# cvg/glue-factory

Hardware: AMD Instinct MI355X
Metric: image-pairs/sec (train step) SP+LightGlue N=2048 d=256 L=9 (higher is better)
Workload: dtype bf16; 1 GPU; configs[1]: SuperPoint + LightGlue train step -- frozen SuperPoint-open forward on 2x32 synthetic 1024x1024 images resident in HBM (view1 = view0 warped by a sampled homography, SURVEY 8(d)(P); first block and the 64-channel 3x3 blocks as fused HIP kernels, library convolutions + fused HIP tails for the 128/256-channel blocks), homography ground truth (gf_gt_nn), LightGlue fwd + loss + bwd + fused; pairs_per_gpu=32, global_batch=32, keypoints=2048, descriptor_dim=256, layers=9, parallelism=dp1

## Files before the change

glue-factory_amd/csrc/conv3x3.hip:

```cpp
#include "gf_common.h"
#include "gf_amd.h"

#ifndef C3_ABL
#define C3_ABL 0
#endif

namespace {

typedef unsigned int u32x4 __attribute__((ext_vector_type(4)));
typedef unsigned int u32x2 __attribute__((ext_vector_type(2)));
typedef __attribute__((address_space(3))) void c3_lds_void;
typedef const __attribute__((address_space(1))) void c3_glb_void;

constexpr int C3_TH = 8, C3_TW = 32;
constexpr int C3_IW = C3_TW + 2, C3_IH = C3_TH + 2;
constexpr int C3_NPIX = C3_IW * C3_IH;
constexpr int C3_PIECES = 44;
constexpr int C3_INBUF = C3_PIECES * 1024;
constexpr int C3_OUT = C3_TH * C3_TW * 128;
constexpr int C3_STAGE = 2 * C3_INBUF;
constexpr int C3_CST = C3_STAGE + 2 * C3_OUT;
constexpr int C3_LDS = C3_CST + 3 * 64 * 4;
#ifndef C3_AGPR_FRAGS_V
#define C3_AGPR_FRAGS_V 48
#endif
constexpr int C3_AGPR_FRAGS = C3_AGPR_FRAGS_V;

template <int OFF> __device__ __forceinline__ u32x4 c3_rd128(unsigned a) {
    u32x4 v;
    asm volatile("ds_read_b128 %0, %1 offset:%2" : "=v"(v) : "v"(a), "n"(OFF) : "memory");
    return v;
}
template <int N> __device__ __forceinline__ void c3_wait_lgkm() { asm volatile("s_waitcnt lgkmcnt(%0)" ::"n"(N) : "memory"); }
template <int N> __device__ __forceinline__ void c3_wait_vm() { asm volatile("s_waitcnt vmcnt(%0)" ::"n"(N) : "memory"); }
template <typename V> __device__ __forceinline__ void c3_tie(V& v) { asm volatile("" : "+v"(v)); }

struct C3Params {
    const bf16_t* x; const bf16_t* w;
    const float* bias; const float* scale; const float* shift;
    bf16_t* y;
    int ldy;
    int B, H, W, relu;
};

template <bool POOL, bool RELU>
__global__ __launch_bounds__(256, 1) void conv3x3_c64_kernel(C3Params p) {
    extern __shared__ __attribute__((aligned(1024))) char smem[];
    const unsigned lds0 = (unsigned)(size_t)smem;
    const int lane = threadIdx.x & 63, wave = __builtin_amdgcn_readfirstlane(threadIdx.x >> 6);
    const int l31 = lane & 31, hi = lane >> 5;
    const int tx_n = p.W / C3_TW, ty_n = p.H / C3_TH;
    const int tiles = tx_n * ty_n * p.B;
#ifndef C3_SKEW32
#define C3_SKEW32 5
#endif
    const int skew = tx_n % 32 == 0 ? C3_SKEW32 : 0;

    bf16x8 wf[2][9][4];
#pragma unroll
    for (int nt = 0; nt < 2; ++nt)
#pragma unroll
        for (int t = 0; t < 9; ++t)
#pragma unroll
            for (int ks = 0; ks < 4; ++ks) {
                const bf16x8 v = *reinterpret_cast<const bf16x8*>(p.w + ((t * 64 + 32 * nt + l31) * 64 + 16 * ks + 8 * hi));
                {
                    wf[nt][t][ks] = v;
                    if ((nt * 9 + t) * 4 + ks < C3_AGPR_FRAGS) asm volatile("" : "+a"(wf[nt][t][ks]));
                    else asm volatile("" : "+v"(wf[nt][t][ks]));
                }
            }
    float* cst = reinterpret_cast<float*>(smem + C3_CST);
    if (threadIdx.x < 64) {
        cst[threadIdx.x] = p.bias[threadIdx.x];
        cst[64 + threadIdx.x] = p.scale[threadIdx.x];
        cst[128 + threadIdx.x] = p.shift[threadIdx.x];
    }

    struct Tile { int b, y0, x0; };
    auto coords = [&](int tile) {
        Tile t;
        t.b = tile / (tx_n * ty_n);
        const int r = tile - t.b * (tx_n * ty_n);
        const int ty = r / tx_n;
        const int tx = (r - ty * tx_n + skew * ty) % tx_n;
        t.y0 = ty * C3_TH; t.x0 = tx * C3_TW;
        return t;
    };
    const int pc_pp0 = wave * 8 + (lane >> 3);
    const int pc_lane0 = pc_pp0 * 128 + ((lane & 7) ^ ((pc_pp0 >> 1) & 7)) * 16;
    const int pc_wrap = (p.W - C3_IW) * 128;
    int pc_off = 0, pc_ix = 0;
    auto image_rsrc = [&](const Tile& t) {
        return __builtin_amdgcn_make_buffer_rsrc((void*)(p.x + (int64_t)t.b * p.H * p.W * 64), 0, p.H * p.W * 128, 0x00020000);
    };
    auto issue_piece = [&](__amdgpu_buffer_rsrc_t rs, const Tile& t, int buf, int i) {
        if (i == 0) { pc_ix = pc_pp0; pc_off = ((t.y0 - 1) * p.W + t.x0 - 1) * 128 + pc_lane0; }
        __builtin_amdgcn_raw_ptr_buffer_load_lds(rs, (c3_lds_void*)(smem + buf * C3_INBUF + (wave + 4 * i) * 1024), 16, pc_off, 0, 0, 0);
        const bool wrap = pc_ix >= C3_IW - 32;
        pc_off += 32 * 128 + (wrap ? pc_wrap : 0);
        pc_ix += wrap ? 32 - C3_IW : 32;
    };
    auto zero_halo = [&](const Tile& t, int buf) {
        for (int pp = threadIdx.x; pp < C3_NPIX; pp += 256) {
            const int iy = pp / C3_IW, ix = pp - iy * C3_IW;
            const int gy = t.y0 - 1 + iy, gx = t.x0 - 1 + ix;
            if (gy < 0 || gy >= p.H || gx < 0 || gx >= p.W) {
                u32x4 z = {0u, 0u, 0u, 0u};
#pragma unroll
                for (int c = 0; c < 8; ++c) *reinterpret_cast<u32x4*>(smem + buf * C3_INBUF + pp * 128 + c * 16) = z;
            }
        }
    };
    auto is_border = [&](const Tile& t) {
        return t.y0 == 0 || t.x0 == 0 || t.y0 == p.H - C3_TH || t.x0 == p.W - C3_TW;
    };

    constexpr int NSTORE = POOL ? 4 : 8;
    const int st_off0 = POOL ? ((int)(threadIdx.x >> 7) * (p.W / 2) + ((int)(threadIdx.x >> 3) & 15)) * p.ldy + ((int)threadIdx.x & 7) * 8
                             : ((int)(threadIdx.x >> 3)) * p.ldy + ((int)threadIdx.x & 7) * 8;
    auto store_addr = [&](const Tile& t, int k) -> bf16_t* {
        if (!POOL) {
            bf16_t* base = p.y + (((int64_t)t.b * p.H + t.y0 + k) * p.W + t.x0) * p.ldy;
            return base + st_off0;
        }
        bf16_t* base = p.y + (((int64_t)t.b * (p.H / 2) + t.y0 / 2 + 2 * k) * (p.W / 2) + t.x0 / 2) * p.ldy;
        return base + st_off0;
    };
    auto stage_at = [&](int sb, int opx, int c) { return C3_STAGE + sb * C3_OUT + opx * 128 + ((c ^ ((opx >> 1) & 7)) << 4); };
    u32x4 sv[POOL ? 2 : 1];
    float pm[POOL ? 8 : 1];
    auto store_read = [&](int sb, int k) {
        if (!POOL) {
            const int u = threadIdx.x + 256 * k;
            sv[0] = c3_rd128<0>(lds0 + stage_at(sb, u >> 3, u & 7));
        } else {
            const int u = threadIdx.x + 256 * (k >> 1);
            const int py = u >> 7, px = (u >> 3) & 15, c = u & 7;
#pragma unroll
            for (int d = 0; d < 2; ++d) sv[d] = c3_rd128<0>(lds0 + stage_at(sb, (2 * py + (k & 1)) * C3_TW + 2 * px + d, c));
        }
    };
    auto store_write = [&](const Tile& t, int k) {
        if (!POOL) {
            c3_tie(sv[0]);
            if (!(C3_ABL & 8)) *reinterpret_cast<u32x4*>(store_addr(t, k)) = sv[0];
        } else {
#pragma unroll
            for (int d = 0; d < 2; ++d) {
                c3_tie(sv[d]);
                const bf16x8 vv = __builtin_bit_cast(bf16x8, sv[d]);
#pragma unroll
                for (int e = 0; e < 8; ++e) pm[e] = (d || (k & 1)) ? fmaxf(pm[e], (float)vv[e]) : (float)vv[e];
            }
            if (k & 1) {
                const bf16x8 o = {(bf16_t)pm[0], (bf16_t)pm[1], (bf16_t)pm[2], (bf16_t)pm[3],
                                  (bf16_t)pm[4], (bf16_t)pm[5], (bf16_t)pm[6], (bf16_t)pm[7]};
                if (!(C3_ABL & 8)) *reinterpret_cast<bf16x8*>(store_addr(t, k >> 1)) = o;
            }
        }
    };

    unsigned ab[4][3];
#pragma unroll
    for (int ro = 0; ro < 4; ++ro)
#pragma unroll
        for (int dx = 0; dx < 3; ++dx) {
            const int pp = (2 * wave + ro) * C3_IW + l31 + dx;
            ab[ro][dx] = lds0 + (unsigned)(pp * 128 + ((hi ^ ((pp >> 1) & 7)) << 4));
        }
    const int T = (tiles - (int)blockIdx.x + (int)gridDim.x - 1) / (int)gridDim.x;
    if (T <= 0) return;
    Tile cur = coords(blockIdx.x), prev = cur;
    {
        const __amdgpu_buffer_rsrc_t rs0 = image_rsrc(cur);
#pragma unroll
        for (int i = 0; i < C3_PIECES / 4; ++i) issue_piece(rs0, cur, 0, i);
    }
    c3_wait_vm<0>();
    asm volatile("s_waitcnt lgkmcnt(0)\n\ts_barrier" ::: "memory");
    if (is_border(cur)) {
        zero_halo(cur, 0);
        asm volatile("s_waitcnt lgkmcnt(0)\n\ts_barrier" ::: "memory");
    }

    for (int i = 0; i < T; ++i) {
        const int buf = i & 1;
        const bool has_next = i + 1 < T;
        const Tile nxt = coords(blockIdx.x + (has_next ? i + 1 : i) * gridDim.x);
        const __amdgpu_buffer_rsrc_t nxt_rs = image_rsrc(nxt);

        f32x16 acc[2][2];
#pragma unroll
        for (int nt = 0; nt < 2; ++nt)
#pragma unroll
            for (int r = 0; r < 2; ++r)
#pragma unroll
                for (int k = 0; k < 16; ++k) acc[nt][r][k] = 0.f;
        auto base = [&](int t, int r) { return ab[r + t / 3][t % 3] + (unsigned)(buf * C3_INBUF); };
        u32x4 ra[4], rb[4];
        if (!(C3_ABL & 4)) {
            const unsigned a = base(0, 0);
#pragma unroll
            for (int ks = 0; ks < 4; ++ks) ra[ks] = c3_rd128<0>(a ^ (32u * ks));
        }
#pragma unroll
        for (int g = 0; g < ((C3_ABL & 4) ? 0 : 18); ++g) {
            const int t = g >> 1, r = g & 1;
            u32x4 (&cur_)[4] = (g & 1) ? rb : ra;
            u32x4 (&nxt_)[4] = (g & 1) ? ra : rb;
            const int k = POOL ? ((g & 3) == 1 && g < 16 ? g >> 2 : -1) : (g >= 1 && g <= 8 ? g - 1 : -1);
            if (k >= 0) store_read(buf ^ 1, k);
            if (g + 1 < 18) {
                const unsigned a = base((g + 1) >> 1, (g + 1) & 1);
#pragma unroll
                for (int ks = 0; ks < 4; ++ks) nxt_[ks] = c3_rd128<0>(a ^ (32u * ks));
                c3_wait_lgkm<4>();
            } else {
                c3_wait_lgkm<0>();
            }
            if (g < C3_PIECES / 4 && !(C3_ABL & 2)) issue_piece(nxt_rs, nxt, buf ^ 1, g);
#pragma unroll
            for (int ks = 0; ks < 4; ++ks) c3_tie(cur_[ks]);
#pragma unroll
            for (int nt = 0; nt < 2; ++nt)
#pragma unroll
                for (int ks = 0; ks < 4; ++ks) {
                    acc[nt][r] = __builtin_amdgcn_mfma_f32_32x32x16_bf16(wf[nt][t][ks], __builtin_bit_cast(bf16x8, cur_[ks]), acc[nt][r], 0, 0, 0);
                }
            if (k >= 0) store_write(prev, k);
        }

        if (C3_ABL & 1) {
#pragma unroll
            for (int r = 0; r < 2; ++r) { asm volatile("" ::"v"(acc[0][r]), "v"(acc[1][r])); }
        } else {
#pragma unroll
            for (int nt = 0; nt < 2; ++nt)
#pragma unroll
                for (int g = 0; g < 4; ++g) {
                    const int c0 = 32 * nt + 8 * g + 4 * hi;
                    const f32x4 cb = *reinterpret_cast<const f32x4*>(cst + c0);
                    const f32x4 cs = *reinterpret_cast<const f32x4*>(cst + 64 + c0);
                    const f32x4 ch = *reinterpret_cast<const f32x4*>(cst + 128 + c0);
#pragma unroll
                    for (int r = 0; r < 2; ++r) {
                        const int opx = (2 * wave + r) * C3_TW + l31;
                        float o[4];
#pragma unroll
                        for (int e = 0; e < 4; ++e) {
                            float a = acc[nt][r][4 * g + e] + cb[e];
                            if (RELU) a = fmaxf(a, 0.f);
                            o[e] = fmaf(a, cs[e], ch[e]);
                        }
                        st4(reinterpret_cast<bf16_t*>(smem + stage_at(buf, opx, 4 * nt + g) + 8 * hi), o[0], o[1], o[2], o[3]);
                    }
                }
        }
        c3_wait_vm<0>();
        asm volatile("s_waitcnt lgkmcnt(0)\n\ts_barrier" ::: "memory");
        if (has_next && is_border(nxt)) {
            zero_halo(nxt, buf ^ 1);
            asm volatile("s_waitcnt lgkmcnt(0)\n\ts_barrier" ::: "memory");
        }
        prev = cur; cur = nxt;
    }
    {
        const int sb = (T - 1) & 1;
#pragma unroll
        for (int k = 0; k < NSTORE; ++k) {
            store_read(sb, k);
            c3_wait_lgkm<0>();
            store_write(prev, k);
        }
    }
}

}

extern "C" int gf_conv3x3_c64_ld(const void* x, const void* w, const float* bias, const float* scale, const float* shift,
                                 void* y, int64_t ldy, int B, int H, int W, int relu, int pool, int dtype, void* stream);
extern "C" int gf_conv3x3_c64(const void* x, const void* w, const float* bias, const float* scale, const float* shift,
                              void* y, int B, int H, int W, int relu, int pool, int dtype, void* stream) {
    return gf_conv3x3_c64_ld(x, w, bias, scale, shift, y, 64, B, H, W, relu, pool, dtype, stream);
}
extern "C" int gf_conv3x3_c64_ld(const void* x, const void* w, const float* bias, const float* scale, const float* shift,
                                 void* y, int64_t ldy, int B, int H, int W, int relu, int pool, int dtype, void* stream) {
    if (B <= 0 || H <= 0 || W <= 0) return GF_ERR_SHAPE;
    if (dtype != GF_BF16) return GF_ERR_DTYPE;
    if (H % C3_TH || W % C3_TW) return GF_ERR_UNSUPPORTED;
    if ((int64_t)H * W * 128 >= (1ll << 31)) return GF_ERR_UNSUPPORTED;
    if (ldy < 64 || ldy % 8) return GF_ERR_ALIGN;
    if ((reinterpret_cast<size_t>(x) | reinterpret_cast<size_t>(w) | reinterpret_cast<size_t>(y)) & 15) return GF_ERR_ALIGN;
    if ((int64_t)H * W * ldy >= (1ll << 31)) return GF_ERR_UNSUPPORTED;
    C3Params p;
    p.x = static_cast<const bf16_t*>(x); p.w = static_cast<const bf16_t*>(w); p.bias = bias; p.scale = scale; p.shift = shift;
    p.y = static_cast<bf16_t*>(y); p.ldy = (int)ldy; p.B = B; p.H = H; p.W = W; p.relu = relu;
    const size_t lds = C3_LDS;
    const int tiles = (W / C3_TW) * (H / C3_TH) * B;
    const int grid = tiles < 256 ? tiles : 256;
    hipStream_t st = reinterpret_cast<hipStream_t>(stream);
    void (*k)(C3Params) = pool ? (relu ? conv3x3_c64_kernel<true, true> : conv3x3_c64_kernel<true, false>)
                               : (relu ? conv3x3_c64_kernel<false, true> : conv3x3_c64_kernel<false, false>);
    hipError_t e = hipFuncSetAttribute(reinterpret_cast<const void*>(k), hipFuncAttributeMaxDynamicSharedMemorySize, (int)lds);
    if (e != hipSuccess) return (int)e;
    k<<<dim3(grid), 256, lds, st>>>(p);
    return (int)hipGetLastError();
}
```

Before: 534.4 image-pairs/s.

## Fuse 2x2 max-pool into conv3x3 epilogue using DPP lane max

For the pooled variant, the 2x2 max-pool now runs in registers inside the epilogue. Vertical max is taken across the two accumulator rows and horizontal max across adjacent lanes via DPP v_max_f32_dpp, and only the pooled result is written to the LDS stage buffer. This quarters stage LDS writes and halves the store loop. The bias/ReLU/scale epilogue math also uses packed f32x2 FMA. It adds inline-asm DPP hazards (s_nop) and changes when pooled stores are issued within the MFMA loop (C3_PG).

Result: no change. 538.7 image-pairs/s, median of 6 (+0.8%).

```diff
diff --git a/glue-factory_amd/csrc/conv3x3.hip b/glue-factory_amd/csrc/conv3x3.hip
--- a/glue-factory_amd/csrc/conv3x3.hip
+++ b/glue-factory_amd/csrc/conv3x3.hip
@@ -21,6 +21,12 @@
 constexpr int C3_STAGE = 2 * C3_INBUF;
 constexpr int C3_CST = C3_STAGE + 2 * C3_OUT;
 constexpr int C3_LDS = C3_CST + 3 * 64 * 4;
+#ifndef C3_PK
+#define C3_PK 1
+#endif
+#ifndef C3_PG
+#define C3_PG 12
+#endif
 #ifndef C3_AGPR_FRAGS_V
 #define C3_AGPR_FRAGS_V 48
 #endif
@@ -34,6 +40,16 @@
 template <int N> __device__ __forceinline__ void c3_wait_lgkm() { asm volatile("s_waitcnt lgkmcnt(%0)" ::"n"(N) : "memory"); }
 template <int N> __device__ __forceinline__ void c3_wait_vm() { asm volatile("s_waitcnt vmcnt(%0)" ::"n"(N) : "memory"); }
 template <typename V> __device__ __forceinline__ void c3_tie(V& v) { asm volatile("" : "+v"(v)); }
+__device__ __forceinline__ void c3_max_lane_xor1(float (&m)[4]) {
+    float r0, r1, r2, r3;
+    asm volatile("s_nop 1\n\t"
+                 "v_max_f32_dpp %0, %4, %4 quad_perm:[1,0,3,2] row_mask:0xf bank_mask:0xf\n\t"
+                 "v_max_f32_dpp %1, %5, %5 quad_perm:[1,0,3,2] row_mask:0xf bank_mask:0xf\n\t"
+                 "v_max_f32_dpp %2, %6, %6 quad_perm:[1,0,3,2] row_mask:0xf bank_mask:0xf\n\t"
+                 "v_max_f32_dpp %3, %7, %7 quad_perm:[1,0,3,2] row_mask:0xf bank_mask:0xf"
+                 : "=&v"(r0), "=&v"(r1), "=&v"(r2), "=&v"(r3) : "v"(m[0]), "v"(m[1]), "v"(m[2]), "v"(m[3]));
+    m[0] = r0; m[1] = r1; m[2] = r2; m[3] = r3;
+}
 
 struct C3Params {
     const bf16_t* x; const bf16_t* w;
@@ -116,7 +132,8 @@
         return t.y0 == 0 || t.x0 == 0 || t.y0 == p.H - C3_TH || t.x0 == p.W - C3_TW;
     };
 
-    constexpr int NSTORE = POOL ? 4 : 8;
+    constexpr int NSTORE = POOL ? 2 : 8;
+    constexpr int OUTB = POOL ? C3_OUT / 4 : C3_OUT;
     const int st_off0 = POOL ? ((int)(threadIdx.x >> 7) * (p.W / 2) + ((int)(threadIdx.x >> 3) & 15)) * p.ldy + ((int)threadIdx.x & 7) * 8
                              : ((int)(threadIdx.x >> 3)) * p.ldy + ((int)threadIdx.x & 7) * 8;
     auto store_addr = [&](const Tile& t, int k) -> bf16_t* {
@@ -127,38 +144,15 @@
         bf16_t* base = p.y + (((int64_t)t.b * (p.H / 2) + t.y0 / 2 + 2 * k) * (p.W / 2) + t.x0 / 2) * p.ldy;
         return base + st_off0;
     };
-    auto stage_at = [&](int sb, int opx, int c) { return C3_STAGE + sb * C3_OUT + opx * 128 + ((c ^ ((opx >> 1) & 7)) << 4); };
-    u32x4 sv[POOL ? 2 : 1];
-    float pm[POOL ? 8 : 1];
+    auto stage_at = [&](int sb, int opx, int c) { return C3_STAGE + sb * OUTB + opx * 128 + ((c ^ ((opx >> 1) & 7)) << 4); };
+    u32x4 sv;
     auto store_read = [&](int sb, int k) {
-        if (!POOL) {
-            const int u = threadIdx.x + 256 * k;
-            sv[0] = c3_rd128<0>(lds0 + stage_at(sb, u >> 3, u & 7));
-        } else {
-            const int u = threadIdx.x + 256 * (k >> 1);
-            const int py = u >> 7, px = (u >> 3) & 15, c = u & 7;
-#pragma unroll
-            for (int d = 0; d < 2; ++d) sv[d] = c3_rd128<0>(lds0 + stage_at(sb, (2 * py + (k & 1)) * C3_TW + 2 * px + d, c));
-        }
+        const int u = threadIdx.x + 256 * k;
+        sv = c3_rd128<0>(lds0 + stage_at(sb, u >> 3, u & 7));
     };
     auto store_write = [&](const Tile& t, int k) {
-        if (!POOL) {
-            c3_tie(sv[0]);
-            if (!(C3_ABL & 8)) *reinterpret_cast<u32x4*>(store_addr(t, k)) = sv[0];
-        } else {
-#pragma unroll
-            for (int d = 0; d < 2; ++d) {
-                c3_tie(sv[d]);
-                const bf16x8 vv = __builtin_bit_cast(bf16x8, sv[d]);
-#pragma unroll
-                for (int e = 0; e < 8; ++e) pm[e] = (d || (k & 1)) ? fmaxf(pm[e], (float)vv[e]) : (float)vv[e];
-            }
-            if (k & 1) {
-                const bf16x8 o = {(bf16_t)pm[0], (bf16_t)pm[1], (bf16_t)pm[2], (bf16_t)pm[3],
-                                  (bf16_t)pm[4], (bf16_t)pm[5], (bf16_t)pm[6], (bf16_t)pm[7]};
-                if (!(C3_ABL & 8)) *reinterpret_cast<bf16x8*>(store_addr(t, k >> 1)) = o;
-            }
-        }
+        c3_tie(sv);
+        if (!(C3_ABL & 8)) *reinterpret_cast<u32x4*>(store_addr(t, k)) = sv;
     };
 
     unsigned ab[4][3];
@@ -209,7 +203,8 @@
             const int t = g >> 1, r = g & 1;
             u32x4 (&cur_)[4] = (g & 1) ? rb : ra;
             u32x4 (&nxt_)[4] = (g & 1) ? ra : rb;
-            const int k = POOL ? ((g & 3) == 1 && g < 16 ? g >> 2 : -1) : (g >= 1 && g <= 8 ? g - 1 : -1);
+            const int g0 = POOL ? C3_PG : 1;
+            const int k = g >= g0 && g < g0 + NSTORE ? g - g0 : -1;
             if (k >= 0) store_read(buf ^ 1, k);
             if (g + 1 < 18) {
                 const unsigned a = base((g + 1) >> 1, (g + 1) & 1);
@@ -235,6 +230,7 @@
 #pragma unroll
             for (int r = 0; r < 2; ++r) { asm volatile("" ::"v"(acc[0][r]), "v"(acc[1][r])); }
         } else {
+            u32x2 pk[POOL ? 8 : 1];
 #pragma unroll
             for (int nt = 0; nt < 2; ++nt)
 #pragma unroll
@@ -243,19 +239,44 @@
                     const f32x4 cb = *reinterpret_cast<const f32x4*>(cst + c0);
                     const f32x4 cs = *reinterpret_cast<const f32x4*>(cst + 64 + c0);
                     const f32x4 ch = *reinterpret_cast<const f32x4*>(cst + 128 + c0);
-#pragma unroll
-                    for (int r = 0; r < 2; ++r) {
-                        const int opx = (2 * wave + r) * C3_TW + l31;
-                        float o[4];
+                    float o[2][4];
+#pragma unroll
+                    for (int r = 0; r < 2; ++r)
+#if !C3_PK
 #pragma unroll
                         for (int e = 0; e < 4; ++e) {
                             float a = acc[nt][r][4 * g + e] + cb[e];
                             if (RELU) a = fmaxf(a, 0.f);
-                            o[e] = fmaf(a, cs[e], ch[e]);
+                            o[r][e] = fmaf(a, cs[e], ch[e]);
                         }
-                        st4(reinterpret_cast<bf16_t*>(smem + stage_at(buf, opx, 4 * nt + g) + 8 * hi), o[0], o[1], o[2], o[3]);
+#else
+#pragma unroll
+                        for (int e = 0; e < 4; e += 2) {
+                            f32x2 a = f32x2{acc[nt][r][4 * g + e], acc[nt][r][4 * g + e + 1]} + f32x2{cb[e], cb[e + 1]};
+                            if (RELU) { a[0] = fmaxf(a[0], 0.f); a[1] = fmaxf(a[1], 0.f); }
+                            a = __builtin_elementwise_fma(a, f32x2{cs[e], cs[e + 1]}, f32x2{ch[e], ch[e + 1]});
+                            o[r][e] = a[0]; o[r][e + 1] = a[1];
+                        }
+#endif
+                    if (!POOL) {
+#pragma unroll
+                        for (int r = 0; r < 2; ++r) {
+                            const int opx = (2 * wave + r) * C3_TW + l31;
+                            st4(reinterpret_cast<bf16_t*>(smem + stage_at(buf, opx, 4 * nt + g) + 8 * hi), o[r][0], o[r][1], o[r][2], o[r][3]);
+                        }
+                    } else {
+#pragma unroll
+                        for (int e = 0; e < 4; ++e) o[0][e] = fmaxf(o[0][e], o[1][e]);
+                        c3_max_lane_xor1(o[0]);
+                        const bf16x4 v = {(bf16_t)o[0][0], (bf16_t)o[0][1], (bf16_t)o[0][2], (bf16_t)o[0][3]};
+                        pk[4 * nt + g] = __builtin_bit_cast(u32x2, v);
                     }
                 }
+            if (POOL && !(lane & 1)) {
+                const int opx = wave * (C3_TW / 2) + (l31 >> 1);
+#pragma unroll
+                for (int c = 0; c < 8; ++c) *reinterpret_cast<u32x2*>(smem + stage_at(buf, opx, c) + 8 * hi) = pk[c];
+            }
         }
         c3_wait_vm<0>();
         asm volatile("s_waitcnt lgkmcnt(0)\n\ts_barrier" ::: "memory");
```
